# theartful/polychase

Measured on AMD Instinct MI355X. Metric: optical-flow frames/sec, higher is better.
Workload: dtype u8/int32 fixed-point + f32 2x2 solve; 1 GPU; C2 1920x1080 300-frame synthetic clip, 3-level pyramidal LK (max_level=3); width=1920, height=1080, max_level=3, window=10, pairs_per_frame=8, frames_per_gpu=1877, arith=opencv_x86, parallelism=single GPU

## Files before the change

### polychase_amd/csrc/hip/api.hip

```cpp
#include "api_internal.hpp"

#include <dirent.h>
#include <unistd.h>

#include <cstring>
#include <mutex>

namespace pc {
std::string& last_error() {
    thread_local std::string e;
    return e;
}
}

namespace pc_api {

int collect_timing(pc_context* c) {
    if (c->ranges.empty()) return PC_OK;
    PC_HIP(c->sync_side_streams());
    PC_HIP(hipStreamSynchronize(c->stream));
    std::vector<std::pair<float, float>> spans[PC_K_COUNT];
    hipEvent_t const origin = c->ranges.front().a;
    for (auto& r : c->ranges) {
        float ms = 0.f, t0 = 0.f;
// ... 91 lines not shown

int validate_gftt(const pc_gftt_options* opt, int w, int h, pc::GfttGrid* g) {
    if (!(opt->quality_level > 0 && opt->min_distance >= 0 && opt->max_corners >= 0))
        return fail(PC_E_INVALID, "GFTT options violate quality_level > 0 && min_distance >= 0 && max_corners >= 0");
    if (opt->gradient_size != 3 && opt->gradient_size != 5 && opt->gradient_size != 7 && opt->gradient_size != -1)
        return fail(PC_E_INVALID, "gradient_size must be 3, 5, 7 (Sobel) or -1 (Scharr)");
    if (opt->block_size < 1) return fail(PC_E_INVALID, "block_size must be >= 1");
    g->rows = std::max(1, opt->grid_rows);
    g->cols = std::max(1, opt->grid_cols);
    if (g->rows * g->cols > pc::kMaxGridCells) return fail(PC_E_INVALID, "grid_rows*grid_cols must be <= %d", pc::kMaxGridCells);
    g->cell_h = (h + g->rows - 1) / g->rows;
    g->cell_w = (w + g->cols - 1) / g->cols;
    return PC_OK;
}

static int corner_response(pc_context* ctx, const pc_frame* f, DetectScratch& d, const pc::GfttGrid& grid, const pc_gftt_options& opt,
                           uint32_t* cell_max) {
    const int fma = ((ctx->arith & PC_ARITH_SOBEL_FMA) ? 1 : 0) | ((ctx->arith & PC_ARITH_SOBEL_ROW_FMA) ? 2 : 0);
    static const bool force_general = getenv("POLYCHASE_GFTT_GENERAL") && atoi(getenv("POLYCHASE_GFTT_GENERAL")) == 1;
    if (opt.block_size == 3 && opt.gradient_size == 3 && !opt.use_harris && !force_general) {
        pc::launch_min_eig(f->levels[0], d.eig.p, grid, cell_max, fma, ctx->work);
        return PC_OK;
    }
    PC_HIP(d.cov.ensure((size_t)3 * f->w * f->h));
    const bool two_pass = opt.block_size >= pc::kBoxRowsFromBlock;
    if (two_pass) PC_HIP(d.box_rows.ensure((size_t)3 * f->w * f->h));
    if (!pc::launch_corner_response(f->levels[0], d.eig.p, d.cov.p, two_pass ? d.box_rows.p : nullptr, grid, cell_max, opt.block_size, opt.gradient_size, opt.use_harris != 0, opt.harris_k,
                                    fma, ctx->work))
        return fail(PC_E_INVALID, "gradient_size must be 3, 5, 7 (Sobel) or -1 (Scharr)");
    return PC_OK;
}

int detect_reserve(pc_context* ctx, int w, int h, DetectScratch& d) {
    const size_t npx = (size_t)w * h;
    const size_t cand_cap = std::min(npx, npx / 4 + 65536);
    PC_HIP(d.eig.ensure(npx));
    PC_HIP(d.cstate.ensure(npx + 16));
    PC_HIP(d.keys.ensure(cand_cap));
    PC_HIP(d.keys_bucketed.ensure(cand_cap));
    PC_HIP(d.keys_sorted.ensure(cand_cap));
    d.cand_cap = (uint32_t)std::min<size_t>(d.keys.cap, std::min(d.keys_bucketed.cap, d.keys_sorted.cap));
    d.ticket_stride = ticket_stride(w, h, d.cand_cap);
    d.counter_words = kTicketsAt + 3 * (int)d.ticket_stride;
    PC_HIP(d.counters.ensure((size_t)d.counter_words));
    PC_HIP(d.bucket_offsets.ensure(pc::kSortBuckets + 1));
    PC_HIP(d.per_block.ensure((size_t)pc::suppress_num_blocks(d.cand_cap) + 1));
    PC_HIP(d.h_counters.ensure(kHostCells));
    if (!d.ev_b) PC_HIP(hipEventCreateWithFlags(&d.ev_b, hipEventDisableTiming));
    (void)ctx;
    return PC_OK;
}

static int upload_suppression_offsets(pc_context* ctx, const pc_gftt_options& opt) {
    if (!(opt.min_distance >= 1) || ctx->sup_min_distance == opt.min_distance) return PC_OK;
// ... 20 lines not shown

static int ensure_perm_capacity(pc_frame* f, int n) {
    if (f->perm_cap >= n) return PC_OK;
    if (f->d_perm) PC_HIP(hipFree(f->d_perm));
    f->d_perm = nullptr;
    f->perm_cap = 0;
    const int want = std::max(n + n / 2, 1024);
    PC_HIP(hipMalloc(&f->d_perm, (size_t)want * 2 * sizeof(uint32_t)));
    f->perm_cap = want;
    return PC_OK;
}

int detect_enqueue(pc_context* ctx, pc_frame* f, const pc::GfttGrid& grid, const pc_gftt_options& opt, DetectScratch& d,
                   DevBuf<uint32_t>& hist, bool full_launch) {
    const int w = f->w, h = f->h;
    int rc = detect_reserve(ctx, w, h, d);
    if (rc != PC_OK) return rc;
    if ((rc = upload_suppression_offsets(ctx, opt)) != PC_OK) return rc;
    if (f->kp_cap < 4096 && (rc = ensure_kp_capacity(f, 4096)) != PC_OK) return rc;
    if ((rc = ensure_perm_capacity(f, f->kp_cap)) != PC_OK) return rc;
    PC_HIP(hist.ensure((size_t)pc::bin_num_tiles(w, h) + 1));
    uint32_t* const cnt = d.counters.p;
    if (!d.cleared) PC_HIP(hipMemsetAsync(cnt, 0, (size_t)d.counter_words * sizeof(uint32_t), ctx->work));
    uint32_t* const tickets = cnt + kTicketsAt;
    d.cleared = false;
    {
        ScopedTimer t(ctx, PC_K_MINEIG);
        if ((rc = corner_response(ctx, f, d, grid, opt, cnt + kCellMaxAt)) != PC_OK) return rc;
    }
    {
        ScopedTimer t(ctx, PC_K_NMS);
        pc::launch_nms(d.eig.p, w, h, grid, cnt + kCellMaxAt, opt.quality_level, d.keys.p, d.cand_cap, cnt + kCntCand, d.cstate.p,
                       cnt + kCntSortParams, cnt + kHistAt, tickets, d.bucket_offsets.p, hist.p, ctx->work);
    }
    const uint32_t n_launch = (ctx->cand_hint > 0 && !full_launch) ? std::min(ctx->cand_hint, d.cand_cap) : d.cand_cap;
    {
        ScopedTimer t(ctx, PC_K_SORT);
        pc::launch_bucket_sort(d.keys.p, d.cand_cap, n_launch, cnt + kCntCand, cnt + kCntSortParams, d.bucket_offsets.p,
                               cnt + kCursorAt, d.keys_bucketed.p, d.keys_sorted.p, cnt + kCntOverflow, ctx->work);
    }
    const uint32_t limit = opt.max_corners > 0 ? std::min<uint32_t>((uint32_t)opt.max_corners, (uint32_t)f->kp_cap) : (uint32_t)f->kp_cap;
    const bool large_radius = opt.min_distance > pc::kSuppressMaxTableRadius;
    if (large_radius) PC_HIP(d.sup_grid.ensure((size_t)pc::suppress_large_grid_words(w, h, opt.min_distance)));
    {
        ScopedTimer t(ctx, PC_K_SUPPRESS);
        pc::launch_suppress_and_compact(d.keys_sorted.p, n_launch, cnt + kCntCand, w, h, d.eig.p, d.cstate.p, ctx->sup_offsets.p,
                                        ctx->n_sup_offsets, ctx->sup_rows.p, ctx->sup_R, opt.min_distance >= 1, d.per_block.p,
                                        cnt + kCntStuck, limit, f->d_kps,
                                        cnt + kCntKps, hist.p, cnt + kCntOverflow, tickets + d.ticket_stride, d.ticket_stride,
                                        opt.min_distance, large_radius ? d.sup_grid.p : nullptr, ctx->work);
    }
    pc::launch_spatial_bins_counted(f->d_kps, (int)std::min<uint32_t>(limit, n_launch), cnt + kCntKps, w, h, hist.p, f->d_perm,
                                    f->d_perm + f->perm_cap, cnt, d.h_counters.p, kHostCells, ctx->work);
    PC_HIP(hipEventRecord(d.ev_b, ctx->work));
    f->n_kps = -1;
    f->n_cands = -1;
    f->perm_valid = false;
    return PC_OK;
}
// ... 846 lines not shown
```

### polychase_amd/csrc/hip/api_analyzer.hip

```cpp
#include "api_internal.hpp"

using namespace pc_api;


namespace {

constexpr int kSpareSlots = PC_ANALYZER_SPARE_SLOTS;

enum DetState { DET_NONE = 0, DET_ENQUEUED = 2, DET_DONE = 3 };

struct Slot {
    pc_frame* frame = nullptr;
    int32_t frame_id = 0;
    bool valid = false;
    DetState det = DET_NONE;
    bool supplied = false;
    DetectScratch scratch;
    hipEvent_t last_read[2] = {nullptr, nullptr};
    hipEvent_t img_ready = nullptr;
    hipEvent_t kps_ready = nullptr;
};

struct Job {
    int32_t frame1 = 0;
// ... 128 lines not shown
    a->grid = grid0;
    a->prio.init();
    a->slots.resize((size_t)ring_frames + kSpareSlots);
    a->jobs.resize((size_t)max_jobs);
    int rc = PC_OK;
    for (auto& s : a->slots) {
        rc = pc_frame_create(ctx, width, height, flow->window_size, flow->max_level, &s.frame);
        if (rc != PC_OK) break;
        const int kp0 = std::max(16384, (width * height) / 16);
        if ((rc = ensure_kp_capacity(s.frame, kp0)) != PC_OK) break;
        if (hipMalloc(reinterpret_cast<void**>(&s.frame->d_perm), (size_t)kp0 * 2 * sizeof(uint32_t)) != hipSuccess) {
            rc = fail(PC_E_HIP, "hipMalloc failed");
            break;
        }
        s.frame->perm_cap = kp0;
        if ((rc = detect_reserve(ctx, width, height, s.scratch)) != PC_OK) break;
        if (s.scratch.bin_hist.ensure((size_t)pc::bin_num_tiles(width, height) + 1) != hipSuccess) {
            rc = fail(PC_E_HIP, "allocation failed");
            break;
        }
        if (hipEventCreateWithFlags(&s.img_ready, hipEventDisableTiming) != hipSuccess ||
            hipEventCreateWithFlags(&s.kps_ready, hipEventDisableTiming) != hipSuccess) {
            rc = fail(PC_E_HIP, "hipEventCreate failed");
            break;
        }
    }
    if (rc == PC_OK)
        for (auto& j : a->jobs)
            if (hipEventCreateWithFlags(&j.done, hipEventDisableTiming) != hipSuccess) {
                rc = fail(PC_E_HIP, "hipEventCreate failed");
                break;
// ... 351 lines not shown
```

### polychase_amd/csrc/hip/api_internal.hpp

```cpp
#pragma once

#include <chrono>
#include <ratio>

#include "internal.hpp"

namespace pc_api {

struct ScopedTimer {
    pc_context* c;
    int cls;
    hipEvent_t a = nullptr, b = nullptr;
    hipStream_t s = nullptr;
    ScopedTimer(pc_context* ctx, int k, hipStream_t on = nullptr) : c(ctx), cls(k), s(on ? on : ctx->work) {
        if (!(c->timing_mask & (1u << k))) return;
        auto get = [&]() {
            hipEvent_t e = nullptr;
            if (!c->event_pool.empty()) {
                e = c->event_pool.back();
                c->event_pool.pop_back();
            } else {
                (void)hipEventCreate(&e);
            }
            return e;
// ... 20 lines not shown

struct SlowSection {
    const char* name;
    std::chrono::steady_clock::time_point t0;
    explicit SlowSection(const char* n) : name(n), t0(std::chrono::steady_clock::now()) {}
    ~SlowSection() {
        if (!pc::trace_allocations()) return;
        const double ms = std::chrono::duration<double, std::milli>(std::chrono::steady_clock::now() - t0).count();
        if (ms > 2.0) fprintf(stderr, "[polychase_hip] slow host section %s: %.2f ms\n", name, ms);
    }
};

int collect_timing(pc_context* c);
int ensure_kp_capacity(pc_frame* f, int n);
int validate_gftt(const pc_gftt_options* opt, int w, int h, pc::GfttGrid* g);
int detect_reserve(pc_context* ctx, int w, int h, DetectScratch& d);
int detect_enqueue(pc_context* ctx, pc_frame* f, const pc::GfttGrid& grid, const pc_gftt_options& opt, DetectScratch& d,
                   DevBuf<uint32_t>& hist, bool full_launch = false);
int detect_finish(pc_context* ctx, pc_frame* f, const pc::GfttGrid& grid, const pc_gftt_options& opt, DetectScratch& d,
                  DevBuf<uint32_t>& hist, bool* redone = nullptr);
int join_prep(pc_context* ctx);
int order_keypoints_spatially(pc_context* ctx, pc_frame* f, DevBuf<uint32_t>& hist);
int check_lk_args(pc_context* ctx, const pc_frame* frame1, const pc_frame* const* targets, int n_targets,
                  const pc_flow_options* opt);
int run_lk(pc_context* ctx, const pc_frame* frame1, const pc_frame* const* targets, int n_targets, const pc_flow_options* opt,
           int set = 0);
int set_image(pc_context* ctx, pc_frame* f, const uint8_t* src, size_t row_pitch, int on_device, int channels, int elem_size = 1,
              uint32_t* clear = nullptr, int clear_words = 0);
int detect_counter_words(const DetectScratch& d);

}
// ... 1 lines not shown
```

### polychase_amd/csrc/hip/internal.hpp

```cpp
#pragma once

#include <hip/hip_runtime.h>

#include <cstdio>
#include <cstdlib>

#include <algorithm>
#include <cmath>
#include <cstdarg>
#include <cstdio>
#include <cstring>
#include <new>
#include <string>
#include <vector>

#include "../../../include/polychase_hip.h"
#include "kernels.hpp"

static_assert(pc::kMaxLevels == PC_MAX_LEVELS, "LKParams holds PC_MAX_LEVELS levels");

namespace pc {

std::string& last_error();

// ... 11 lines not shown
    do {                                                                                          \
        hipError_t e_ = (expr);                                                                   \
        if (e_ != hipSuccess)                                                                     \
            return fail(PC_E_HIP, "%s failed: %s (%s:%d)", #expr, hipGetErrorString(e_), __FILE__, __LINE__); \
    } while (0)

inline bool trace_allocations() {
    static const bool on = getenv("POLYCHASE_TRACE_ALLOC") != nullptr;
    return on;
}

template <typename T>
struct DevBuf {
    T* p = nullptr;
    size_t cap = 0;
    hipError_t ensure(size_t n) {
        if (n <= cap) return hipSuccess;
        if (p) (void)hipFree(p);
        p = nullptr;
        cap = 0;
        size_t want = n + n / 2 + 64;
        if (trace_allocations()) fprintf(stderr, "[polychase_hip] device buffer %zu -> %zu bytes\n", cap * sizeof(T), want * sizeof(T));
        hipError_t e = hipMalloc(reinterpret_cast<void**>(&p), want * sizeof(T));
        if (e == hipSuccess) cap = want;
        return e;
    }
    void release() {
        if (p) (void)hipFree(p);
        p = nullptr;
        cap = 0;
    }
};

template <typename T>
struct PinBuf {
    T* p = nullptr;
// ... 18 lines not shown

struct TimedRange {
    int cls;
    hipEvent_t a, b;
};

}

using pc::DevBuf;
using pc::PinBuf;
using pc::TimedRange;
using pc::fail;

struct DetectScratch {
    DevBuf<unsigned long long> keys, keys_bucketed, keys_sorted;
    DevBuf<float> eig;
    DevBuf<float> cov;
    DevBuf<double> box_rows;
    DevBuf<uint8_t> cstate;
    DevBuf<uint32_t> counters;
    DevBuf<uint32_t> bucket_offsets;
    DevBuf<uint32_t> per_block;
    DevBuf<uint32_t> sup_grid;
    DevBuf<uint32_t> bin_hist;
    PinBuf<uint32_t> h_counters;
    hipEvent_t ev_b = nullptr;
    uint32_t cand_cap = 0;
    int counter_words = 0;
    uint32_t ticket_stride = 0;
    bool cleared = false;
    void release() {
        keys.release();
        keys_bucketed.release();
        keys_sorted.release();
        eig.release();
        cov.release();
        box_rows.release();
        cstate.release();
        counters.release();
        bucket_offsets.release();
        per_block.release();
        sup_grid.release();
        bin_hist.release();
        h_counters.release();
        if (ev_b) (void)hipEventDestroy(ev_b);
        ev_b = nullptr;
    }
};
// ... 78 lines not shown
```

### polychase_amd/csrc/hip/kernels.hpp

```cpp
#pragma once

#include "bvh.hpp"
#include "common.hpp"

namespace pc {

int helper_prio_arg();
void set_helper_prio(int hi);

void launch_rgb2gray(const uint8_t* rgb, size_t rgb_pitch, const Level& l0, hipStream_t s);
void launch_rgbf32_to_gray(const float* rgb, size_t rgb_pitch, int channels, const Level& l0, hipStream_t s);
void launch_copy_gray(const uint8_t* gray, size_t gray_pitch, const Level& l0, hipStream_t s);
void launch_pyrdown(const Level& src, const Level& dst, hipStream_t s);
void launch_border(const Level& l, int win, hipStream_t s);
void launch_widen(const Level& l, int win, hipStream_t s);
void launch_scharr(const Level& l, hipStream_t s);

enum LevelSourceKind { SRC_PYR = 0, SRC_RGB8 = 1, SRC_GRAY8 = 2, SRC_RGBF32 = 3 };
struct LevelSource {
    int kind;
    const uint8_t* src;
    size_t src_pitch;
    int channels;
    int aligned;
// ... 1 lines not shown
    uint32_t* clear;
    int clear_words;
};
void launch_level(const LevelSource& in, const Level& out, int win, hipStream_t s);

struct GfttGrid {
    int rows, cols;
    int cell_w, cell_h;
};
constexpr int kMaxGridCells = 1024;
void launch_min_eig(const Level& l0, float* eig, const GfttGrid& g, uint32_t* cell_max, int sobel_fma, hipStream_t s);
constexpr int kBoxRowsFromBlock = 12;
bool launch_corner_response(const Level& l0, float* eig, float* cov, double* box_rows, const GfttGrid& g, uint32_t* cell_max, int block_size, int gradient_size,
                            bool harris, double harris_k, int sobel_fma, hipStream_t s);
constexpr int kSortBuckets = 8192;
void launch_nms(const float* eig, int w, int h, const GfttGrid& g, const uint32_t* cell_max, double quality_level,
                unsigned long long* keys, uint32_t cap, uint32_t* counter, uint8_t* cstate, uint32_t* sort_params, uint32_t* hist,
                uint32_t* ticket, uint32_t* bucket_offsets, uint32_t* bin_hist, hipStream_t s);
void launch_bucket_sort(const unsigned long long* keys, uint32_t cap, uint32_t n_launch, const uint32_t* counter, const uint32_t* sort_params,
                        const uint32_t* offsets, uint32_t* cursor, unsigned long long* scratch, unsigned long long* out,
                        uint32_t* overflow, hipStream_t s);
int suppress_num_blocks(uint32_t n);
void launch_suppress_and_compact(const unsigned long long* keys, uint32_t n_max, const uint32_t* n_dev, int w, int h, const float* eig,
                                 uint8_t* cstate, const int2* offsets, int n_offsets, const int* row_hw, int R, bool suppress,
                                 uint32_t* per_block,
                                 uint32_t* stuck, uint32_t max_corners, float2* xy, uint32_t* n_out, uint32_t* bin_hist,
                                 uint32_t* overflow, uint32_t* tickets, uint32_t ticket_stride, double large_min_distance, uint32_t* large_grid,
                                 hipStream_t s);
constexpr double kSuppressMaxTableRadius = 64.0;
int suppress_large_grid_words(int w, int h, double min_distance);
hipError_t sort_keys_desc(void* temp, size_t& temp_bytes, unsigned long long* keys_in,
                          unsigned long long* keys_out, uint32_t n, hipStream_t s);

constexpr int kMaxLevels = 16;
struct LKParams {
    Level src[kMaxLevels];
    const uint8_t* tgt[8][kMaxLevels];
    const uint16_t* tgt16[8][kMaxLevels];
    int n_targets;
    int max_level;
    int n;
    const float2* pts;
    const uint32_t* perm;
// ... 151 lines not shown
```

### polychase_amd/csrc/hip/kernels_gftt.hip

```cpp
#include <algorithm>
#include <cstring>
#include <type_traits>
#include <rocprim/device/device_radix_sort.hpp>

#include <cmath>

#include "kernels.hpp"

namespace pc {

constexpr int TW = 64, TH = 16;
constexpr int GH = TH + 4, G_PITCH = 72;
constexpr int CW = TW + 2, CH = TH + 2;

template <bool ROW_FMA>
__device__ __forceinline__ float smooth_row(float a, float b, float c, float f1, float f0) {
    float t = f1 * a;
    if (ROW_FMA) {
        t = __fmaf_rn(f0, b, t);
        t = __fmaf_rn(f1, c, t);
    } else {
        t += f0 * b;
        t += f1 * c;
    }
// ... 512 lines not shown
    while ((span >> r.shift) >= (uint32_t)kSortBuckets) r.shift++;
    return r;
}
__device__ __forceinline__ uint32_t bucket_of(uint32_t ord, const SortRange& r) {
    const uint32_t d = r.hi > ord ? r.hi - ord : 0u;
    const uint32_t b = d >> r.shift;
    return b < (uint32_t)kSortBuckets ? b : (uint32_t)kSortBuckets - 1u;
}

__global__ __launch_bounds__(256) void nms_kernel(const float* __restrict__ eig, int w, int h, GfttGrid g,
                                                  const uint32_t* __restrict__ cell_max, double quality_level,
                                                  unsigned long long* __restrict__ keys, uint32_t cap,
                                                  uint32_t* __restrict__ counter, uint8_t* __restrict__ cstate,
                                                  uint32_t* __restrict__ sort_params, uint32_t* __restrict__ hist,
                                                  uint32_t* __restrict__ ticket, uint32_t* __restrict__ bucket_offsets,
                                                  uint32_t* __restrict__ bin_hist, int n_tiles, int hi_prio) {
    helper_priority(hi_prio);
    __shared__ float s_thr[kMaxGridCells];
    __shared__ uint32_t s_hi, s_lo;
    __shared__ float s_v[CH][CW + 2];
    __shared__ uint32_t s_wave[4];
    __shared__ uint32_t s_base;
    const int tid = threadIdx.x;
    const int x0 = blockIdx.x * TW;
    const int ncells = g.rows * g.cols;
    if (tid == 0) {
        s_hi = 0u;
        s_lo = 0xffffffffu;
    }
    __syncthreads();
    for (int i = tid; i < ncells; i += 256) {
        const float mx = ordered_to_float(cell_max[i]);
        s_thr[i] = (float)((double)mx * quality_level);
        atomicMax(&s_hi, cell_max[i]);
        atomicMin(&s_lo, float_to_ordered(s_thr[i] > 0.f ? s_thr[i] : 0.f));
    }
    __syncthreads();
    const SortRange range = make_sort_range(s_lo, s_hi);
    if (blockIdx.x == 0 && blockIdx.y == 0) {
        if (tid == 0) {
            sort_params[0] = range.hi;
            sort_params[1] = range.shift;
        }
        if (bin_hist)
            for (int i = tid; i < n_tiles; i += 256) bin_hist[i] = 0u;
    }
    const int r = tid >> 4, q = tid & 15;
    const int x = x0 + 4 * q;
    uint32_t flags = 0;
    float vals[NMS_SUB][4];
#pragma unroll
    for (int sub = 0; sub < NMS_SUB; sub++) {
        const int y0 = (blockIdx.y * NMS_SUB + sub) * TH;
        const int y = y0 + r;
        __syncthreads();
        const bool big_cells = g.cell_w >= CW && g.cell_h >= CH;
        const int ccx0 = max(x0 - 1, 0) / g.cell_w, ccy0 = max(y0 - 1, 0) / g.cell_h;
        const int bx = (ccx0 + 1) * g.cell_w, by = (ccy0 + 1) * g.cell_h;
        auto thr_at = [&](int ax, int ay) -> float {
            const int cx = big_cells ? ccx0 + (ax >= bx) : ax / g.cell_w;
            const int cy = big_cells ? ccy0 + (ay >= by) : ay / g.cell_h;
// ... 79 lines not shown
        const uint32_t total = s_wave[0] + s_wave[1] + s_wave[2] + s_wave[3];
        s_base = total ? atomicAdd(counter, total) : 0u;
    }
    __syncthreads();
    if (cnt != 0) {
        uint32_t pos = s_base + incl - cnt;
        for (int wv = 0; wv < wave; wv++) pos += s_wave[wv];
#pragma unroll
        for (int sub = 0; sub < NMS_SUB; sub++) {
            const int y = (blockIdx.y * NMS_SUB + sub) * TH + r;
#pragma unroll
            for (int i = 0; i < 4; i++) {
                if (flags & (1u << (4 * sub + i))) {
                    const uint32_t ord = float_to_ordered(vals[sub][i]);
                    if (pos < cap) {
                        keys[pos] = ((unsigned long long)ord << 32) | (unsigned long long)(uint32_t)(y * w + x + i);
                        atomicAdd(&hist[bucket_of(ord, range)], 1u);
                    }
                    pos++;
                }
            }
        }
    }
    if (ticket && last_workgroup(ticket, gridDim.x * gridDim.y)) {
        __shared__ uint32_t s_scan[256];
        const uint32_t total = scan_exclusive_256_fixed<kSortBuckets / 256>(hist, bucket_offsets, s_scan);
        if (tid == 0) bucket_offsets[kSortBuckets] = total;
    }
}

void launch_nms(const float* eig, int w, int h, const GfttGrid& g, const uint32_t* cell_max, double quality_level,
                unsigned long long* keys, uint32_t cap, uint32_t* counter, uint8_t* cstate, uint32_t* sort_params, uint32_t* hist,
                uint32_t* ticket, uint32_t* bucket_offsets, uint32_t* bin_hist, hipStream_t s) {
    dim3 grid((w + TW - 1) / TW, (h + NMS_SUB * TH - 1) / (NMS_SUB * TH));
    hipLaunchKernelGGL(nms_kernel, grid, dim3(256), 0, s, eig, w, h, g, cell_max, quality_level, keys, cap, counter, cstate,
                       sort_params, hist, ticket, bucket_offsets, bin_hist, bin_hist ? bin_num_tiles(w, h) : 0, helper_prio_arg());
}

constexpr int kBucketLds = 512;

__global__ __launch_bounds__(256) void bucket_scatter_kernel(const unsigned long long* __restrict__ keys, uint32_t cap,
                                                             const uint32_t* __restrict__ counter, const uint32_t* __restrict__ sort_params,
                                                             const uint32_t* __restrict__ offsets, uint32_t* __restrict__ cursor,
                                                             unsigned long long* __restrict__ out, int hi_prio) {
    helper_priority(hi_prio);
    const uint32_t n = min(*counter, cap);
    SortRange range;
    range.hi = sort_params[0];
    range.shift = sort_params[1];
    for (uint32_t i = blockIdx.x * blockDim.x + threadIdx.x; i < n; i += gridDim.x * blockDim.x) {
        const unsigned long long key = keys[i];
        const uint32_t b = bucket_of((uint32_t)(key >> 32), range);
        out[offsets[b] + atomicAdd(&cursor[b], 1u)] = key;
    }
}

constexpr int kBucketsPerWave = 4;

constexpr int kSortWaves = 4;
__global__ __launch_bounds__(64 * kSortWaves) void bucket_sort_kernel(const unsigned long long* __restrict__ in, const uint32_t* __restrict__ offsets,
                                                         unsigned long long* __restrict__ out, uint32_t* __restrict__ overflow, int hi_prio) {
    helper_priority(hi_prio);
    __shared__ unsigned long long s_all[kSortWaves][kBucketLds];
    const int lane = threadIdx.x & 63, wave = threadIdx.x >> 6;
    unsigned long long* const s_keys = s_all[wave];
    const int b0 = (blockIdx.x * kSortWaves + wave) * kBucketsPerWave;
    if (b0 >= kSortBuckets) return;
    uint32_t o[kBucketsPerWave + 1];
#pragma unroll
    for (int k = 0; k <= kBucketsPerWave; k++) o[k] = offsets[min(b0 + k, kSortBuckets)];
    const uint32_t lo = o[0], n4 = o[kBucketsPerWave] - lo;
    if (n4 == 0) return;
    if (n4 <= (uint32_t)kBucketLds) {
        unsigned long long ld[kBucketLds / 64];
#pragma unroll
        for (int q = 0; q < kBucketLds / 64; q++) {
            const uint32_t i = lane + 64 * q;
            ld[q] = i < n4 ? in[lo + i] : 0ull;
        }
#pragma unroll
        for (int q = 0; q < kBucketLds / 64; q++) {
            const uint32_t i = lane + 64 * q;
            if (i < n4) s_keys[i] = ld[q];
        }
        __builtin_amdgcn_fence(__ATOMIC_ACQ_REL, "wavefront");
        uint32_t longest = 0;
#pragma unroll
        for (int k = 0; k < kBucketsPerWave; k++) longest = max(longest, o[k + 1] - o[k]);
        for (uint32_t i = lane; i < n4; i += 64) {
            const unsigned long long mine = s_keys[i];
            uint32_t a = lo, b = o[1];
#pragma unroll
            for (int k = 1; k < kBucketsPerWave; k++)
// ... 2 lines not shown
                    b = o[k + 1];
                }
            const uint32_t first = a - lo, len = b - a;
            uint32_t rank = 0;
#pragma unroll 8
            for (uint32_t j = 0; j < longest; j++) {
                const unsigned long long other = s_keys[first + min(j, len - 1u)];
                rank += (j < len && other > mine) ? 1u : 0u;
            }
            out[a + rank] = mine;
        }
        return;
    }
    for (int b = b0; b < b0 + kBucketsPerWave && b < kSortBuckets; b++) {
        const uint32_t base = offsets[b], n = offsets[b + 1] - base;
        if (n == 0) continue;
        if (n > (uint32_t)kBucketLds) {
            if (lane == 0) atomicOr(overflow, 1u);
            for (uint32_t i = lane; i < n; i += 64) out[base + i] = in[base + i];
            continue;
        }
        __builtin_amdgcn_fence(__ATOMIC_ACQ_REL, "wavefront");
        for (uint32_t i = lane; i < n; i += 64) s_keys[i] = in[base + i];
        __builtin_amdgcn_fence(__ATOMIC_ACQ_REL, "wavefront");
        for (uint32_t i = lane; i < n; i += 64) {
            const unsigned long long mine = s_keys[i];
            uint32_t rank = 0;
#pragma unroll 8
            for (uint32_t j = 0; j < n; j++) rank += s_keys[j] > mine ? 1u : 0u;
            out[base + rank] = mine;
        }
    }
}

void launch_bucket_sort(const unsigned long long* keys, uint32_t cap, uint32_t n_launch, const uint32_t* counter, const uint32_t* sort_params,
                        const uint32_t* offsets, uint32_t* cursor, unsigned long long* scratch, unsigned long long* out,
                        uint32_t* overflow, hipStream_t s) {
    const unsigned blocks = std::max(1u, std::min<unsigned>(1024u, (n_launch + 255u) / 256u));
    hipLaunchKernelGGL(bucket_scatter_kernel, dim3(blocks), dim3(256), 0, s, keys, cap, counter, sort_params, offsets, cursor, scratch, helper_prio_arg());
    hipLaunchKernelGGL(bucket_sort_kernel, dim3((kSortBuckets / kBucketsPerWave + kSortWaves - 1) / kSortWaves), dim3(64 * kSortWaves), 0, s, scratch, offsets,
                       out, overflow, helper_prio_arg());
}

struct AcceptedScan {
    uint32_t* ticket;
    uint32_t* n_out;
    uint32_t* overflow;
    uint32_t max_corners;
};
__device__ __forceinline__ void finish_accepted_scan(uint32_t* per_block, const AcceptedScan& fin, uint32_t n_max, const uint32_t* n_dev) {
    if (!last_workgroup(fin.ticket, gridDim.x)) return;
    __shared__ uint32_t s_scan[256];
    if (threadIdx.x == 0 && n_dev && fin.overflow && *n_dev > n_max) atomicOr(fin.overflow, 4u);
    const uint32_t total = scan_exclusive_256(per_block, per_block, (int)gridDim.x, s_scan);
    if (threadIdx.x == 0) *fin.n_out = (fin.max_corners > 0 && total > fin.max_corners) ? fin.max_corners : total;
}

constexpr uint8_t CS_CAND = 1, CS_ACCEPTED = 2, CS_REJECTED = 3;
constexpr int SUP_NB = 12;
constexpr int SUP_BLOCK = 256;

__device__ __forceinline__ uint8_t cs_load(const uint8_t* p) { return __hip_atomic_load(p, __ATOMIC_RELAXED, __HIP_MEMORY_SCOPE_AGENT); }
__device__ __forceinline__ void cs_store(uint8_t* p, uint8_t v) { __hip_atomic_store(p, v, __ATOMIC_RELAXED, __HIP_MEMORY_SCOPE_AGENT); }

__global__ __launch_bounds__(SUP_BLOCK) void suppress_sorted_kernel(const unsigned long long* __restrict__ keys, uint32_t n_max,
                                                                    const uint32_t* __restrict__ n_dev, int w, int h,
                                                                    const float* __restrict__ eig, uint8_t* cstate,
                                                                    const int2* __restrict__ offsets, int n_offsets,
                                                                    const int* __restrict__ row_hw, int R,
                                                                    uint32_t* __restrict__ accepted_per_block,
                                                                    uint32_t* __restrict__ stuck, AcceptedScan fin, int hi_prio) {
    helper_priority(hi_prio);
    const uint32_t n = n_dev ? min(*n_dev, n_max) : n_max;
    const uint32_t i = blockIdx.x * SUP_BLOCK + threadIdx.x;
    const bool live = i < n;
    uint32_t my_val = 0, my_idx = 0;
    uint32_t nb[SUP_NB];
    int n_nb = 0;
    bool overflow = false;
    int x = 0, y = 0;
    if (live) {
        const unsigned long long key = keys[i];
        my_val = (uint32_t)(key >> 32);
        my_idx = (uint32_t)key;
        y = (int)(my_idx / (uint32_t)w);
        x = (int)(my_idx - (uint32_t)y * (uint32_t)w);
        for (int dy = -R; dy <= R; dy++) {
            const int ny = y + dy, hw = row_hw[dy + R];
// ... 50 lines not shown
                }
            }
            if (rejected || !blocked) {
                cs_store(&cstate[my_idx], rejected ? CS_REJECTED : CS_ACCEPTED);
                accepted = !rejected;
                done = true;
            }
        }
        if (__all(done)) break;
        if (spin > (1u << 22)) {
            if (!done) atomicAdd(stuck, 1u);
            break;
        }
        __builtin_amdgcn_s_sleep(1);
    }
    const int c = __syncthreads_count(accepted);
    if (threadIdx.x == 0) publish(&accepted_per_block[blockIdx.x], (uint32_t)c);
    finish_accepted_scan(accepted_per_block, fin, n_max, n_dev);
}

__global__ __launch_bounds__(SUP_BLOCK) void accept_all_kernel(const unsigned long long* __restrict__ keys, uint32_t n_max,
                                                               const uint32_t* __restrict__ n_dev, uint8_t* cstate,
                                                               uint32_t* __restrict__ accepted_per_block, AcceptedScan fin, int hi_prio) {
    helper_priority(hi_prio);
    const uint32_t n = n_dev ? min(*n_dev, n_max) : n_max;
    const uint32_t i = blockIdx.x * SUP_BLOCK + threadIdx.x;
    if (i < n) cstate[(uint32_t)keys[i]] = CS_ACCEPTED;
    const uint32_t first = blockIdx.x * SUP_BLOCK;
    if (threadIdx.x == 0) publish(&accepted_per_block[blockIdx.x], first < n ? min((uint32_t)SUP_BLOCK, n - first) : 0u);
    finish_accepted_scan(accepted_per_block, fin, n_max, n_dev);
}

__global__ __launch_bounds__(SUP_BLOCK) void accepted_scatter_kernel(const unsigned long long* __restrict__ keys, uint32_t n_max,
// ... 133 lines not shown
    if (suppress && large_grid) {
        const int cell = suppress_large_cell(w, h, large_min_distance), gw = (w + cell - 1) / cell, gh = (h + cell - 1) / cell;
        (void)hipMemsetAsync(large_grid, 0, (size_t)gw * gh * kLargeCellWords * sizeof(uint32_t), s);
        hipLaunchKernelGGL(suppress_large_radius_kernel, dim3(1), dim3(256), 0, s, keys, n_max, n_dev, w, cstate, large_min_distance * large_min_distance,
                           cell, gw, gh, large_grid, accepted_per_block, nb, stuck, n_out, overflow, max_corners, helper_prio_arg());
    } else if (suppress)
        hipLaunchKernelGGL(suppress_sorted_kernel, dim3(nb), dim3(SUP_BLOCK), 0, s, keys, n_max, n_dev, w, h, eig, cstate, offsets,
                           n_offsets, row_hw, R, accepted_per_block, stuck, fin, helper_prio_arg());
    else
        hipLaunchKernelGGL(accept_all_kernel, dim3(nb), dim3(SUP_BLOCK), 0, s, keys, n_max, n_dev, cstate, accepted_per_block, fin, helper_prio_arg());
    const int tiles_x = (w + 63) >> 6, n_tiles = bin_hist ? bin_num_tiles(w, h) : 0;
    hipLaunchKernelGGL(accepted_scatter_kernel, dim3(nb), dim3(SUP_BLOCK), 0, s, keys, n_max, n_dev, w, cstate, per_block, max_corners, xy,
                       bin_hist, tiles_x, n_tiles, tickets + ticket_stride, helper_prio_arg());
}

hipError_t sort_keys_desc(void* temp, size_t& temp_bytes, unsigned long long* keys_in,
                          unsigned long long* keys_out, uint32_t n, hipStream_t s) {
    return rocprim::radix_sort_keys_desc(temp, temp_bytes, keys_in, keys_out, (size_t)n, 0u, 64u, s);
}

}
```

Baseline: 3286 frames/s.

## Fuse GFTT detection: NMS writes bucket slots, single-pass suppress-compact with lookback

On the default fast path (3x3 min-eig, table-sized min_distance), NMS now scatters candidate keys straight into fixed per-bucket slots, so the separate bucket scatter pass is dropped and the sort reads the slots directly. Suppression and compaction are merged into one kernel that uses a decoupled-lookback prefix scan instead of a separate scatter kernel. NMS also zeroes the lookback array, which saves a memset. This cuts kernel launches and global passes in detection. In exchange it adds a fixed slot buffer and spin-wait lookback, and overflow falls back through the existing redo path.

```diff
diff --git a/polychase_amd/csrc/hip/api.hip b/polychase_amd/csrc/hip/api.hip
--- a/polychase_amd/csrc/hip/api.hip
+++ b/polychase_amd/csrc/hip/api.hip
@@ -129,11 +129,19 @@
     return PC_OK;
 }
 
+static bool tiled_response(const pc_gftt_options& opt) {
+    static const bool force_general = getenv("POLYCHASE_GFTT_GENERAL") && atoi(getenv("POLYCHASE_GFTT_GENERAL")) == 1;
+    return opt.block_size == 3 && opt.gradient_size == 3 && !opt.use_harris && !force_general;
+}
+
+static bool fused_detection(const pc_gftt_options& opt) {
+    return tiled_response(opt) && opt.min_distance >= 1 && !(opt.min_distance > pc::kSuppressMaxTableRadius);
+}
+
 static int corner_response(pc_context* ctx, const pc_frame* f, DetectScratch& d, const pc::GfttGrid& grid, const pc_gftt_options& opt,
                            uint32_t* cell_max) {
     const int fma = ((ctx->arith & PC_ARITH_SOBEL_FMA) ? 1 : 0) | ((ctx->arith & PC_ARITH_SOBEL_ROW_FMA) ? 2 : 0);
-    static const bool force_general = getenv("POLYCHASE_GFTT_GENERAL") && atoi(getenv("POLYCHASE_GFTT_GENERAL")) == 1;
-    if (opt.block_size == 3 && opt.gradient_size == 3 && !opt.use_harris && !force_general) {
+    if (tiled_response(opt)) {
         pc::launch_min_eig(f->levels[0], d.eig.p, grid, cell_max, fma, ctx->work);
         return PC_OK;
     }
@@ -146,13 +154,14 @@
     return PC_OK;
 }
 
-int detect_reserve(pc_context* ctx, int w, int h, DetectScratch& d) {
+int detect_reserve(pc_context* ctx, int w, int h, DetectScratch& d, const pc_gftt_options* opt) {
     const size_t npx = (size_t)w * h;
     const size_t cand_cap = std::min(npx, npx / 4 + 65536);
     PC_HIP(d.eig.ensure(npx));
     PC_HIP(d.cstate.ensure(npx + 16));
     PC_HIP(d.keys.ensure(cand_cap));
     PC_HIP(d.keys_bucketed.ensure(cand_cap));
+    if (opt && fused_detection(*opt)) PC_HIP(d.key_slots.ensure((size_t)pc::kSortBuckets * pc::kBucketSlots, true));
     PC_HIP(d.keys_sorted.ensure(cand_cap));
     d.cand_cap = (uint32_t)std::min<size_t>(d.keys.cap, std::min(d.keys_bucketed.cap, d.keys_sorted.cap));
     d.ticket_stride = ticket_stride(w, h, d.cand_cap);
@@ -203,7 +212,7 @@
 int detect_enqueue(pc_context* ctx, pc_frame* f, const pc::GfttGrid& grid, const pc_gftt_options& opt, DetectScratch& d,
                    DevBuf<uint32_t>& hist, bool full_launch) {
     const int w = f->w, h = f->h;
-    int rc = detect_reserve(ctx, w, h, d);
+    int rc = detect_reserve(ctx, w, h, d, &opt);
     if (rc != PC_OK) return rc;
     if ((rc = upload_suppression_offsets(ctx, opt)) != PC_OK) return rc;
     if (f->kp_cap < 4096 && (rc = ensure_kp_capacity(f, 4096)) != PC_OK) return rc;
@@ -213,6 +222,9 @@
     if (!d.cleared) PC_HIP(hipMemsetAsync(cnt, 0, (size_t)d.counter_words * sizeof(uint32_t), ctx->work));
     uint32_t* const tickets = cnt + kTicketsAt;
     d.cleared = false;
+    const uint32_t n_launch = (ctx->cand_hint > 0 && !full_launch) ? std::min(ctx->cand_hint, d.cand_cap) : d.cand_cap;
+    const bool large_radius = opt.min_distance > pc::kSuppressMaxTableRadius;
+    const bool fused = fused_detection(opt);
     {
         ScopedTimer t(ctx, PC_K_MINEIG);
         if ((rc = corner_response(ctx, f, d, grid, opt, cnt + kCellMaxAt)) != PC_OK) return rc;
@@ -220,18 +232,25 @@
     {
         ScopedTimer t(ctx, PC_K_NMS);
         pc::launch_nms(d.eig.p, w, h, grid, cnt + kCellMaxAt, opt.quality_level, d.keys.p, d.cand_cap, cnt + kCntCand, d.cstate.p,
-                       cnt + kCntSortParams, cnt + kHistAt, tickets, d.bucket_offsets.p, hist.p, ctx->work);
-    }
-    const uint32_t n_launch = (ctx->cand_hint > 0 && !full_launch) ? std::min(ctx->cand_hint, d.cand_cap) : d.cand_cap;
+                       cnt + kCntSortParams, cnt + kHistAt, tickets, d.bucket_offsets.p, hist.p, ctx->work,
+                       fused ? d.key_slots.p : nullptr, fused ? d.per_block.p : nullptr, pc::suppress_num_blocks(n_launch));
+    }
     {
         ScopedTimer t(ctx, PC_K_SORT);
-        pc::launch_bucket_sort(d.keys.p, d.cand_cap, n_launch, cnt + kCntCand, cnt + kCntSortParams, d.bucket_offsets.p,
-                               cnt + kCursorAt, d.keys_bucketed.p, d.keys_sorted.p, cnt + kCntOverflow, ctx->work);
+        if (fused)
+            pc::launch_bucket_sort_slots(d.key_slots.p, d.bucket_offsets.p, d.keys_sorted.p, cnt + kCntOverflow, ctx->work);
+        else
+            pc::launch_bucket_sort(d.keys.p, d.cand_cap, n_launch, cnt + kCntCand, cnt + kCntSortParams, d.bucket_offsets.p,
+                                   cnt + kCursorAt, d.keys_bucketed.p, d.keys_sorted.p, cnt + kCntOverflow, ctx->work);
     }
     const uint32_t limit = opt.max_corners > 0 ? std::min<uint32_t>((uint32_t)opt.max_corners, (uint32_t)f->kp_cap) : (uint32_t)f->kp_cap;
-    const bool large_radius = opt.min_distance > pc::kSuppressMaxTableRadius;
     if (large_radius) PC_HIP(d.sup_grid.ensure((size_t)pc::suppress_large_grid_words(w, h, opt.min_distance)));
-    {
+    if (fused) {
+        ScopedTimer t(ctx, PC_K_SUPPRESS);
+        pc::launch_suppress_compact(d.keys_sorted.p, n_launch, cnt + kCntCand, w, h, d.eig.p, d.cstate.p, ctx->sup_offsets.p,
+                                    ctx->n_sup_offsets, ctx->sup_rows.p, ctx->sup_R, d.per_block.p, cnt + kCntStuck, limit, f->d_kps,
+                                    cnt + kCntKps, hist.p, cnt + kCntOverflow, tickets + d.ticket_stride, ctx->work);
+    } else {
         ScopedTimer t(ctx, PC_K_SUPPRESS);
         pc::launch_suppress_and_compact(d.keys_sorted.p, n_launch, cnt + kCntCand, w, h, d.eig.p, d.cstate.p, ctx->sup_offsets.p,
                                         ctx->n_sup_offsets, ctx->sup_rows.p, ctx->sup_R, opt.min_distance >= 1, d.per_block.p,
diff --git a/polychase_amd/csrc/hip/api_analyzer.hip b/polychase_amd/csrc/hip/api_analyzer.hip
--- a/polychase_amd/csrc/hip/api_analyzer.hip
+++ b/polychase_amd/csrc/hip/api_analyzer.hip
@@ -166,7 +166,7 @@
             break;
         }
         s.frame->perm_cap = kp0;
-        if ((rc = detect_reserve(ctx, width, height, s.scratch)) != PC_OK) break;
+        if ((rc = detect_reserve(ctx, width, height, s.scratch, &a->gopt)) != PC_OK) break;
         if (s.scratch.bin_hist.ensure((size_t)pc::bin_num_tiles(width, height) + 1) != hipSuccess) {
             rc = fail(PC_E_HIP, "allocation failed");
             break;
diff --git a/polychase_amd/csrc/hip/api_internal.hpp b/polychase_amd/csrc/hip/api_internal.hpp
--- a/polychase_amd/csrc/hip/api_internal.hpp
+++ b/polychase_amd/csrc/hip/api_internal.hpp
@@ -58,7 +58,7 @@
 int collect_timing(pc_context* c);
 int ensure_kp_capacity(pc_frame* f, int n);
 int validate_gftt(const pc_gftt_options* opt, int w, int h, pc::GfttGrid* g);
-int detect_reserve(pc_context* ctx, int w, int h, DetectScratch& d);
+int detect_reserve(pc_context* ctx, int w, int h, DetectScratch& d, const pc_gftt_options* opt = nullptr);
 int detect_enqueue(pc_context* ctx, pc_frame* f, const pc::GfttGrid& grid, const pc_gftt_options& opt, DetectScratch& d,
                    DevBuf<uint32_t>& hist, bool full_launch = false);
 int detect_finish(pc_context* ctx, pc_frame* f, const pc::GfttGrid& grid, const pc_gftt_options& opt, DetectScratch& d,
diff --git a/polychase_amd/csrc/hip/internal.hpp b/polychase_amd/csrc/hip/internal.hpp
--- a/polychase_amd/csrc/hip/internal.hpp
+++ b/polychase_amd/csrc/hip/internal.hpp
@@ -49,12 +49,12 @@
 struct DevBuf {
     T* p = nullptr;
     size_t cap = 0;
-    hipError_t ensure(size_t n) {
+    hipError_t ensure(size_t n, bool exact = false) {
         if (n <= cap) return hipSuccess;
         if (p) (void)hipFree(p);
         p = nullptr;
         cap = 0;
-        size_t want = n + n / 2 + 64;
+        size_t want = exact ? n : n + n / 2 + 64;
         if (trace_allocations()) fprintf(stderr, "[polychase_hip] device buffer %zu -> %zu bytes\n", cap * sizeof(T), want * sizeof(T));
         hipError_t e = hipMalloc(reinterpret_cast<void**>(&p), want * sizeof(T));
         if (e == hipSuccess) cap = want;
@@ -103,6 +103,7 @@
 
 struct DetectScratch {
     DevBuf<unsigned long long> keys, keys_bucketed, keys_sorted;
+    DevBuf<unsigned long long> key_slots;
     DevBuf<float> eig;
     DevBuf<float> cov;
     DevBuf<double> box_rows;
@@ -121,6 +122,7 @@
     void release() {
         keys.release();
         keys_bucketed.release();
+        key_slots.release();
         keys_sorted.release();
         eig.release();
         cov.release();
diff --git a/polychase_amd/csrc/hip/kernels.hpp b/polychase_amd/csrc/hip/kernels.hpp
--- a/polychase_amd/csrc/hip/kernels.hpp
+++ b/polychase_amd/csrc/hip/kernels.hpp
@@ -39,12 +39,16 @@
 bool launch_corner_response(const Level& l0, float* eig, float* cov, double* box_rows, const GfttGrid& g, uint32_t* cell_max, int block_size, int gradient_size,
                             bool harris, double harris_k, int sobel_fma, hipStream_t s);
 constexpr int kSortBuckets = 8192;
+constexpr int kBucketSlots = 512;
 void launch_nms(const float* eig, int w, int h, const GfttGrid& g, const uint32_t* cell_max, double quality_level,
                 unsigned long long* keys, uint32_t cap, uint32_t* counter, uint8_t* cstate, uint32_t* sort_params, uint32_t* hist,
-                uint32_t* ticket, uint32_t* bucket_offsets, uint32_t* bin_hist, hipStream_t s);
+                uint32_t* ticket, uint32_t* bucket_offsets, uint32_t* bin_hist, hipStream_t s,
+                unsigned long long* slots = nullptr, uint32_t* zero = nullptr, int zero_words = 0);
 void launch_bucket_sort(const unsigned long long* keys, uint32_t cap, uint32_t n_launch, const uint32_t* counter, const uint32_t* sort_params,
                         const uint32_t* offsets, uint32_t* cursor, unsigned long long* scratch, unsigned long long* out,
                         uint32_t* overflow, hipStream_t s);
+void launch_bucket_sort_slots(const unsigned long long* slots, const uint32_t* offsets, unsigned long long* out, uint32_t* overflow,
+                              hipStream_t s);
 int suppress_num_blocks(uint32_t n);
 void launch_suppress_and_compact(const unsigned long long* keys, uint32_t n_max, const uint32_t* n_dev, int w, int h, const float* eig,
                                  uint8_t* cstate, const int2* offsets, int n_offsets, const int* row_hw, int R, bool suppress,
@@ -52,6 +56,10 @@
                                  uint32_t* stuck, uint32_t max_corners, float2* xy, uint32_t* n_out, uint32_t* bin_hist,
                                  uint32_t* overflow, uint32_t* tickets, uint32_t ticket_stride, double large_min_distance, uint32_t* large_grid,
                                  hipStream_t s);
+void launch_suppress_compact(const unsigned long long* keys, uint32_t n_max, const uint32_t* n_dev, int w, int h, const float* eig,
+                             uint8_t* cstate, const int2* offsets, int n_offsets, const int* row_hw, int R, uint32_t* lookback,
+                             uint32_t* stuck, uint32_t max_corners, float2* xy, uint32_t* n_out, uint32_t* bin_hist,
+                             uint32_t* overflow, uint32_t* ticket, hipStream_t s);
 constexpr double kSuppressMaxTableRadius = 64.0;
 int suppress_large_grid_words(int w, int h, double min_distance);
 hipError_t sort_keys_desc(void* temp, size_t& temp_bytes, unsigned long long* keys_in,
diff --git a/polychase_amd/csrc/hip/kernels_gftt.hip b/polychase_amd/csrc/hip/kernels_gftt.hip
--- a/polychase_amd/csrc/hip/kernels_gftt.hip
+++ b/polychase_amd/csrc/hip/kernels_gftt.hip
@@ -550,7 +550,9 @@
                                                   uint32_t* __restrict__ counter, uint8_t* __restrict__ cstate,
                                                   uint32_t* __restrict__ sort_params, uint32_t* __restrict__ hist,
                                                   uint32_t* __restrict__ ticket, uint32_t* __restrict__ bucket_offsets,
-                                                  uint32_t* __restrict__ bin_hist, int n_tiles, int hi_prio) {
+                                                  uint32_t* __restrict__ bin_hist, int n_tiles,
+                                                  unsigned long long* __restrict__ slots, uint32_t* __restrict__ zero, int zero_words,
+                                                  int hi_prio) {
     helper_priority(hi_prio);
     __shared__ float s_thr[kMaxGridCells];
     __shared__ uint32_t s_hi, s_lo;
@@ -581,6 +583,7 @@
         if (bin_hist)
             for (int i = tid; i < n_tiles; i += 256) bin_hist[i] = 0u;
     }
+    for (int i = (blockIdx.y * gridDim.x + blockIdx.x) * 256 + tid; i < zero_words; i += gridDim.x * gridDim.y * 256) zero[i] = 0u;
     const int r = tid >> 4, q = tid & 15;
     const int x = x0 + 4 * q;
     uint32_t flags = 0;
@@ -690,8 +693,15 @@
                 if (flags & (1u << (4 * sub + i))) {
                     const uint32_t ord = float_to_ordered(vals[sub][i]);
                     if (pos < cap) {
-                        keys[pos] = ((unsigned long long)ord << 32) | (unsigned long long)(uint32_t)(y * w + x + i);
-                        atomicAdd(&hist[bucket_of(ord, range)], 1u);
+                        const unsigned long long key = ((unsigned long long)ord << 32) | (unsigned long long)(uint32_t)(y * w + x + i);
+                        const uint32_t b = bucket_of(ord, range);
+                        if (slots) {
+                            const uint32_t at = atomicAdd(&hist[b], 1u);
+                            slots[(size_t)b * kBucketSlots + min(at, (uint32_t)kBucketSlots - 1u)] = key;
+                        } else {
+                            keys[pos] = key;
+                            atomicAdd(&hist[b], 1u);
+                        }
                     }
                     pos++;
                 }
@@ -707,10 +717,12 @@
 
 void launch_nms(const float* eig, int w, int h, const GfttGrid& g, const uint32_t* cell_max, double quality_level,
                 unsigned long long* keys, uint32_t cap, uint32_t* counter, uint8_t* cstate, uint32_t* sort_params, uint32_t* hist,
-                uint32_t* ticket, uint32_t* bucket_offsets, uint32_t* bin_hist, hipStream_t s) {
+                uint32_t* ticket, uint32_t* bucket_offsets, uint32_t* bin_hist, hipStream_t s,
+                unsigned long long* slots, uint32_t* zero, int zero_words) {
     dim3 grid((w + TW - 1) / TW, (h + NMS_SUB * TH - 1) / (NMS_SUB * TH));
     hipLaunchKernelGGL(nms_kernel, grid, dim3(256), 0, s, eig, w, h, g, cell_max, quality_level, keys, cap, counter, cstate,
-                       sort_params, hist, ticket, bucket_offsets, bin_hist, bin_hist ? bin_num_tiles(w, h) : 0, helper_prio_arg());
+                       sort_params, hist, ticket, bucket_offsets, bin_hist, bin_hist ? bin_num_tiles(w, h) : 0, slots, zero,
+                       zero ? zero_words : 0, helper_prio_arg());
 }
 
 constexpr int kBucketLds = 512;
@@ -734,6 +746,8 @@
 constexpr int kBucketsPerWave = 4;
 
 constexpr int kSortWaves = 4;
+static_assert(kBucketSlots == kBucketLds, "a bucket beyond its slots is a bucket beyond the fast path");
+template <bool SLOTS>
 __global__ __launch_bounds__(64 * kSortWaves) void bucket_sort_kernel(const unsigned long long* __restrict__ in, const uint32_t* __restrict__ offsets,
                                                          unsigned long long* __restrict__ out, uint32_t* __restrict__ overflow, int hi_prio) {
     helper_priority(hi_prio);
@@ -752,7 +766,15 @@
 #pragma unroll
         for (int q = 0; q < kBucketLds / 64; q++) {
             const uint32_t i = lane + 64 * q;
-            ld[q] = i < n4 ? in[lo + i] : 0ull;
+            size_t at = lo + i;
+            if (SLOTS) {
+                int k = 0;
+#pragma unroll
+                for (int kk = 1; kk < kBucketsPerWave; kk++)
+                    if (lo + i >= o[kk]) k = kk;
+                at = (size_t)(b0 + k) * kBucketSlots + (lo + i - o[k]);
+            }
+            ld[q] = i < n4 ? in[at] : 0ull;
         }
 #pragma unroll
         for (int q = 0; q < kBucketLds / 64; q++) {
@@ -785,14 +807,15 @@
     }
     for (int b = b0; b < b0 + kBucketsPerWave && b < kSortBuckets; b++) {
         const uint32_t base = offsets[b], n = offsets[b + 1] - base;
+        const unsigned long long* const src = SLOTS ? in + (size_t)b * kBucketSlots : in + base;
         if (n == 0) continue;
         if (n > (uint32_t)kBucketLds) {
             if (lane == 0) atomicOr(overflow, 1u);
-            for (uint32_t i = lane; i < n; i += 64) out[base + i] = in[base + i];
+            for (uint32_t i = lane; i < n; i += 64) out[base + i] = src[SLOTS ? min(i, (uint32_t)kBucketSlots - 1u) : i];
             continue;
         }
         __builtin_amdgcn_fence(__ATOMIC_ACQ_REL, "wavefront");
-        for (uint32_t i = lane; i < n; i += 64) s_keys[i] = in[base + i];
+        for (uint32_t i = lane; i < n; i += 64) s_keys[i] = src[i];
         __builtin_amdgcn_fence(__ATOMIC_ACQ_REL, "wavefront");
         for (uint32_t i = lane; i < n; i += 64) {
             const unsigned long long mine = s_keys[i];
@@ -809,8 +832,13 @@
                         uint32_t* overflow, hipStream_t s) {
     const unsigned blocks = std::max(1u, std::min<unsigned>(1024u, (n_launch + 255u) / 256u));
     hipLaunchKernelGGL(bucket_scatter_kernel, dim3(blocks), dim3(256), 0, s, keys, cap, counter, sort_params, offsets, cursor, scratch, helper_prio_arg());
-    hipLaunchKernelGGL(bucket_sort_kernel, dim3((kSortBuckets / kBucketsPerWave + kSortWaves - 1) / kSortWaves), dim3(64 * kSortWaves), 0, s, scratch, offsets,
-                       out, overflow, helper_prio_arg());
+    hipLaunchKernelGGL(bucket_sort_kernel<false>, dim3((kSortBuckets / kBucketsPerWave + kSortWaves - 1) / kSortWaves), dim3(64 * kSortWaves), 0, s, scratch,
+                       offsets, out, overflow, helper_prio_arg());
+}
+void launch_bucket_sort_slots(const unsigned long long* slots, const uint32_t* offsets, unsigned long long* out, uint32_t* overflow,
+                              hipStream_t s) {
+    hipLaunchKernelGGL(bucket_sort_kernel<true>, dim3((kSortBuckets / kBucketsPerWave + kSortWaves - 1) / kSortWaves), dim3(64 * kSortWaves), 0, s, slots,
+                       offsets, out, overflow, helper_prio_arg());
 }
 
 struct AcceptedScan {
@@ -834,15 +862,10 @@
 __device__ __forceinline__ uint8_t cs_load(const uint8_t* p) { return __hip_atomic_load(p, __ATOMIC_RELAXED, __HIP_MEMORY_SCOPE_AGENT); }
 __device__ __forceinline__ void cs_store(uint8_t* p, uint8_t v) { __hip_atomic_store(p, v, __ATOMIC_RELAXED, __HIP_MEMORY_SCOPE_AGENT); }
 
-__global__ __launch_bounds__(SUP_BLOCK) void suppress_sorted_kernel(const unsigned long long* __restrict__ keys, uint32_t n_max,
-                                                                    const uint32_t* __restrict__ n_dev, int w, int h,
-                                                                    const float* __restrict__ eig, uint8_t* cstate,
-                                                                    const int2* __restrict__ offsets, int n_offsets,
-                                                                    const int* __restrict__ row_hw, int R,
-                                                                    uint32_t* __restrict__ accepted_per_block,
-                                                                    uint32_t* __restrict__ stuck, AcceptedScan fin, int hi_prio) {
-    helper_priority(hi_prio);
-    const uint32_t n = n_dev ? min(*n_dev, n_max) : n_max;
+__device__ __forceinline__ bool suppress_decide(const unsigned long long* __restrict__ keys, uint32_t n, int w, int h,
+                                                const float* __restrict__ eig, uint8_t* cstate, const int2* __restrict__ offsets,
+                                                int n_offsets, const int* __restrict__ row_hw, int R, uint32_t* __restrict__ stuck,
+                                                uint32_t* idx_out) {
     const uint32_t i = blockIdx.x * SUP_BLOCK + threadIdx.x;
     const bool live = i < n;
     uint32_t my_val = 0, my_idx = 0;
@@ -923,9 +946,112 @@
         }
         __builtin_amdgcn_s_sleep(1);
     }
+    *idx_out = my_idx;
+    return accepted;
+}
+
+__global__ __launch_bounds__(SUP_BLOCK) void suppress_sorted_kernel(const unsigned long long* __restrict__ keys, uint32_t n_max,
+                                                                    const uint32_t* __restrict__ n_dev, int w, int h,
+                                                                    const float* __restrict__ eig, uint8_t* cstate,
+                                                                    const int2* __restrict__ offsets, int n_offsets,
+                                                                    const int* __restrict__ row_hw, int R,
+                                                                    uint32_t* __restrict__ accepted_per_block,
+                                                                    uint32_t* __restrict__ stuck, AcceptedScan fin, int hi_prio) {
+    helper_priority(hi_prio);
+    const uint32_t n = n_dev ? min(*n_dev, n_max) : n_max;
+    uint32_t idx;
+    const bool accepted = suppress_decide(keys, n, w, h, eig, cstate, offsets, n_offsets, row_hw, R, stuck, &idx);
     const int c = __syncthreads_count(accepted);
     if (threadIdx.x == 0) publish(&accepted_per_block[blockIdx.x], (uint32_t)c);
     finish_accepted_scan(accepted_per_block, fin, n_max, n_dev);
+}
+
+constexpr uint32_t kLbAggregate = 1u << 30, kLbPrefix = 1u << 31, kLbCount = kLbAggregate - 1u;
+__device__ __forceinline__ uint32_t lookback_exclusive(uint32_t* lookback, uint32_t b, uint32_t c, uint32_t* __restrict__ stuck) {
+    const int lane = (int)(threadIdx.x & 63);
+    if (b == 0) {
+        if (lane == 0) publish(&lookback[0], kLbPrefix | c);
+        return 0u;
+    }
+    if (lane == 0) publish(&lookback[b], kLbAggregate | c);
+    uint32_t excl = 0;
+    int top = (int)b - 1;
+    for (uint32_t spin = 0;; spin++) {
+        const int j = top - lane;
+        const uint32_t v = j >= 0 ? __hip_atomic_load(&lookback[j], __ATOMIC_RELAXED, __HIP_MEMORY_SCOPE_AGENT) : kLbPrefix;
+        const unsigned long long pre = __ballot((v & kLbPrefix) != 0u);
+        const int stop = pre ? __ffsll((long long)pre) - 1 : 63;
+        const unsigned long long upto = stop == 63 ? ~0ull : ((2ull << stop) - 1ull);
+        if ((__ballot(v == 0u) & upto) == 0ull) {
+            uint32_t part = lane <= stop ? (v & kLbCount) : 0u;
+#pragma unroll
+            for (int d = 32; d >= 1; d >>= 1) part += __shfl_xor(part, d);
+            excl += part;
+            if (pre) break;
+            top -= 64;
+            continue;
+        }
+        if (spin > (1u << 22)) {
+            if (lane == 0) atomicAdd(stuck, 1u);
+            break;
+        }
+        __builtin_amdgcn_s_sleep(1);
+    }
+    if (lane == 0) publish(&lookback[b], kLbPrefix | (excl + c));
+    return excl;
+}
+
+__global__ __launch_bounds__(SUP_BLOCK) void suppress_compact_kernel(const unsigned long long* __restrict__ keys, uint32_t n_max,
+                                                                     const uint32_t* __restrict__ n_dev, int w, int h,
+                                                                     const float* __restrict__ eig, uint8_t* cstate,
+                                                                     const int2* __restrict__ offsets, int n_offsets,
+                                                                     const int* __restrict__ row_hw, int R, uint32_t* lookback,
+                                                                     uint32_t* __restrict__ stuck, uint32_t max_corners,
+                                                                     float2* __restrict__ xy, uint32_t* __restrict__ n_out,
+                                                                     uint32_t* __restrict__ bin_hist, int tiles_x, int n_tiles,
+                                                                     uint32_t* __restrict__ overflow, uint32_t* __restrict__ ticket,
+                                                                     int hi_prio) {
+    helper_priority(hi_prio);
+    __shared__ uint32_t s_wave[SUP_BLOCK / 64];
+    __shared__ uint32_t s_excl;
+    const uint32_t n_all = n_dev ? *n_dev : n_max;
+    const bool redo = (overflow && (*overflow & 1u) != 0u) || n_all > n_max;
+    const uint32_t n = redo ? 0u : n_all;
+    if (blockIdx.x * SUP_BLOCK < n) {
+        uint32_t idx;
+        const bool accepted = suppress_decide(keys, n, w, h, eig, cstate, offsets, n_offsets, row_hw, R, stuck, &idx);
+        const unsigned long long ballot = __ballot(accepted);
+        const int lane = threadIdx.x & 63, wave = threadIdx.x >> 6;
+        if (lane == 0) s_wave[wave] = (uint32_t)__popcll(ballot);
+        __syncthreads();
+        if (wave == 0) {
+            uint32_t c = 0;
+#pragma unroll
+            for (int wv = 0; wv < SUP_BLOCK / 64; wv++) c += s_wave[wv];
+            const uint32_t excl = lookback_exclusive(lookback, blockIdx.x, c, stuck);
+            if (lane == 0) s_excl = excl;
+        }
+        __syncthreads();
+        if (accepted) {
+            uint32_t pos = s_excl + (uint32_t)__popcll(ballot & ((1ull << lane) - 1ull));
+            for (int wv = 0; wv < wave; wv++) pos += s_wave[wv];
+            if (!(max_corners > 0 && pos >= max_corners)) {
+                const uint32_t y = idx / (uint32_t)w, x = idx - y * (uint32_t)w;
+                xy[pos] = make_float2((float)x, (float)y);
+                if (bin_hist) atomicAdd(&bin_hist[min(n_tiles - 1, (int)((y >> 6) * tiles_x + (x >> 6)))], 1u);
+            }
+        }
+    }
+    if (last_workgroup(ticket, gridDim.x)) {
+        __shared__ uint32_t s_scan[256];
+        if (threadIdx.x == 0) {
+            const uint32_t total =
+                n ? (__hip_atomic_load(&lookback[(n - 1u) / SUP_BLOCK], __ATOMIC_RELAXED, __HIP_MEMORY_SCOPE_AGENT) & kLbCount) : 0u;
+            *n_out = (max_corners > 0 && total > max_corners) ? max_corners : total;
+            if (n_dev && overflow && *n_dev > n_max) atomicOr(overflow, 4u);
+        }
+        if (bin_hist) (void)scan_exclusive_256(bin_hist, bin_hist, n_tiles, s_scan);
+    }
 }
 
 __global__ __launch_bounds__(SUP_BLOCK) void accept_all_kernel(const unsigned long long* __restrict__ keys, uint32_t n_max,
@@ -1089,6 +1215,17 @@
                        bin_hist, tiles_x, n_tiles, tickets + ticket_stride, helper_prio_arg());
 }
 
+void launch_suppress_compact(const unsigned long long* keys, uint32_t n_max, const uint32_t* n_dev, int w, int h, const float* eig,
+                             uint8_t* cstate, const int2* offsets, int n_offsets, const int* row_hw, int R, uint32_t* lookback,
+                             uint32_t* stuck, uint32_t max_corners, float2* xy, uint32_t* n_out, uint32_t* bin_hist,
+                             uint32_t* overflow, uint32_t* ticket, hipStream_t s) {
+    const int nb = suppress_num_blocks(n_max);
+    if (nb == 0) return;
+    const int tiles_x = (w + 63) >> 6, n_tiles = bin_hist ? bin_num_tiles(w, h) : 0;
+    hipLaunchKernelGGL(suppress_compact_kernel, dim3(nb), dim3(SUP_BLOCK), 0, s, keys, n_max, n_dev, w, h, eig, cstate, offsets, n_offsets,
+                       row_hw, R, lookback, stuck, max_corners, xy, n_out, bin_hist, tiles_x, n_tiles, overflow, ticket, helper_prio_arg());
+}
+
 hipError_t sort_keys_desc(void* temp, size_t& temp_bytes, unsigned long long* keys_in,
                           unsigned long long* keys_out, uint32_t n, hipStream_t s) {
     return rocprim::radix_sort_keys_desc(temp, temp_bytes, keys_in, keys_out, (size_t)n, 0u, 64u, s);
```

New measurement: 3407 frames/s (median of 6 runs). +3.7%, better.
